# BarisYazici/deep-rl-grasping

Measured on NVIDIA H100. Metric: SAC grad-steps/sec (batch 256, 64x64 depth), higher is better.
Workload: dtype bf16x3 (fp32-faithful split, f32 accumulate)

## Files before the change

### deep-rl-grasping_b200/csrc/cg.cu

```cuda
#include <cuda_bf16.h>

#include <cstdio>
#include <cstdlib>

#include "cg.cuh"
#include "common.cuh"
#include "wgmma.cuh"

namespace b2g {
namespace {

constexpr int NEPI_WARPS = CG_EPI_WARPS, NPROD_WARPS = 2, PROD_WARP0 = NEPI_WARPS;
constexpr int NTHREADS = 32 * (NEPI_WARPS + 4);
constexpr int PROD_REGS = 40, CONS_REGS = 232;
constexpr int STG_BYTES = 2 * 64 * 16 * 4;

__device__ __forceinline__ uint32_t smem_u32(const void* p) { return (uint32_t)__cvta_generic_to_shared(p); }
__device__ __forceinline__ void mbar_init(uint32_t bar, uint32_t count) {
  asm volatile("mbarrier.init.shared::cta.b64 [%0], %1;" ::"r"(bar), "r"(count));
}
__device__ __forceinline__ void mbar_arrive(uint32_t bar) { asm volatile("mbarrier.arrive.shared::cta.b64 _, [%0];" ::"r"(bar) : "memory"); }
__device__ __forceinline__ void mbar_expect_tx(uint32_t bar, uint32_t bytes) {
  asm volatile("mbarrier.arrive.expect_tx.shared::cta.b64 _, [%0], %1;" ::"r"(bar), "r"(bytes) : "memory");
}
__device__ __forceinline__ void mbar_wait(uint32_t bar, uint32_t parity) {
  asm volatile(
      "{\n\t"
      ".reg .pred p;\n\t"
      "CG_WAIT:\n\t"
// ... 117 lines not shown
__device__ __forceinline__ void stamp_if(long long* dst, bool pred) {
  asm volatile(
      "{\n\t"
      ".reg .pred p;\n\t"
      ".reg .u64 t;\n\t"
      "mov.u64 t, %%clock64;\n\t"
      "setp.ne.u32 p, %1, 0;\n\t"
      "@p st.global.u64 [%0], t;\n\t"
      "}" ::"l"(dst), "r"((uint32_t)pred)
      : "memory");
}

template <int NT, int NPROD, int TRANS, int KS, class Body>
__device__ __forceinline__ void consume_tile(const CgProblem& P, const Tile& ti, uint32_t ring, uint32_t stg, int slot_bytes, int nstages, uint32_t& s,
                                             uint32_t& ph, uint64_t* bar_full, uint64_t* bar_empty, bool nomma, long long* ctrace, uint32_t& gc,
                                             Body&& body) {
  constexpr int NGRP = NPROD >= 6 ? 3 : (NPROD >= 3 ? 2 : 1);
  constexpr int NACC = NT / 2 * NGRP;
  const int tid = threadIdx.x, lane = tid & 31, warp = tid >> 5;
  const int wg = warp >> 2, wl = warp & 3, half = wl >> 1;
  float acc[NACC];
#pragma unroll
  for (int j = 0; j < NACC; ++j) acc[j] = 0.f;
  const uint32_t a_ps = (uint32_t)P.a_pstride, b_ps = (uint32_t)P.b_pstride, a_off = P.a_off, b_off = P.b_off, a_ks = P.a_kstep, b_ks = P.b_kstep;
  const uint32_t a_lbo = P.a_lbo, b_lbo = P.b_lbo;
  const uint32_t m_off = TRANS ? (uint32_t)wg * a_lbo : (uint32_t)wg * 8192u;
  uint32_t prev = 0;
  if (nomma) {
    for (int c = ti.c_begin; c < ti.c_end; ++c, ++gc) {
      mbar_wait(smem_u32(&bar_full[s]), (ph >> s) & 1u);
      mbar_arrive_if(smem_u32(&bar_empty[s]), lane == 0);
// ... 15 lines not shown
      stamp_if(tr + 5, stamp);
      prev = s;
      ph ^= 1u << s;
      if (++s == (uint32_t)nstages) s = 0;
    }
    wg_wait<0>();
    mbar_arrive_if(smem_u32(&bar_empty[prev]), lane == 0);
  }
  if constexpr (NGRP > 2) {
#pragma unroll
    for (int j = 0; j < NT / 2; ++j) acc[j] = acc[j] + (acc[j + NT / 2] + acc[j + NT]);
  } else if constexpr (NGRP > 1) {
#pragma unroll
    for (int j = 0; j < NT / 2; ++j) acc[j] = acc[j] + acc[j + NT / 2];
  }
  const int rrow = 32 * (wl & 1) + lane;
  const uint32_t wstg = stg + (uint32_t)wg * 4096u;
#pragma unroll
  for (int R = 0; R < (NT + 63) / 64; ++R) {
    float x[32];
#pragma unroll
    for (int t = 0; t < 4; ++t) {
      const int c0 = 64 * R + 16 * t;
      if (c0 < NT) {
        asm volatile("bar.sync %0, 128;" ::"r"(1 + wg) : "memory");
#pragma unroll
        for (int jj = 0; jj < 2; ++jj)
#pragma unroll
          for (int h = 0; h < 2; ++h) {
            const int row = 16 * wl + (lane >> 2) + 8 * h, chunk = 2 * jj + ((lane & 3) >> 1);
// ... 5 lines not shown
        if (half == (t >> 1)) {
#pragma unroll
          for (int cc = 0; cc < 4; ++cc) {
            const uint32_t a = wstg + (uint32_t)rrow * 64u + (uint32_t)((cc ^ ((rrow >> 1) & 3)) << 4);
            float* xd = x + 16 * (t & 1) + 4 * cc;
            asm volatile("ld.shared.v4.f32 {%0,%1,%2,%3}, [%4];" : "=f"(xd[0]), "=f"(xd[1]), "=f"(xd[2]), "=f"(xd[3]) : "r"(a));
          }
        }
      }
    }
    const int g = 2 * R + half;
    if (32 * g < NT) body(g, x);
  }
}

__global__ void __launch_bounds__(NTHREADS, 1)
cg_kernel(const __grid_constant__ CgPack pk, int nprob, int total_tiles, const CUtensorMap* __restrict__ maps, int max_stages,
          int dbg, long long* __restrict__ trace) {
  const CgProblem* __restrict__ probs = pk.p;
  extern __shared__ uint8_t smem_raw[];
  __shared__ __align__(8) uint64_t bar_full[CG_MAX_STAGES], bar_empty[CG_MAX_STAGES];
  const int tid = threadIdx.x, lane = tid & 31;
  const int warp = __shfl_sync(0xffffffffu, tid >> 5, 0);
  const int trace_cta = dbg >> 8;
  const bool dbg_noload = dbg & 1, dbg_nomma = dbg & 2, dbg_nostore = dbg & 4, dbg_nost = dbg & 16;
  if (tid == 0) {
    for (int s = 0; s < max_stages; ++s) { mbar_init(smem_u32(&bar_full[s]), 1); mbar_init(smem_u32(&bar_empty[s]), NEPI_WARPS); }
    asm volatile("fence.mbarrier_init.release.cluster;" ::: "memory");
  }
  __syncthreads();
  const uint32_t stg = (smem_u32(smem_raw) + 1023u) & ~1023u;
  const uint32_t ring = stg + STG_BYTES;
  pdl_trigger();
  pdl_wait();

  if (warp >= PROD_WARP0) {
    asm volatile("setmaxnreg.dec.sync.aligned.u32 %0;" ::"n"(PROD_REGS));
    const int pw = warp - PROD_WARP0;
    if (pw >= NPROD_WARPS) return;
    {
      uint32_t gc = 0, s = 0, ph = 0;
      int slot_bytes = 0, nstages = 1;
      Walker w;
      int n2 = 1, nloads = 0, planes = 0, tx = 0;
      const int* tab = nullptr;
      for (int tile = blockIdx.x; tile < total_tiles; tile += gridDim.x) {
        if (w.advance(probs, nprob, tile)) {
          const CgProblem& P = probs[w.p];
          n2 = P.n2; nloads = P.nloads; planes = P.planes; tx = P.tx_bytes; tab = P.tm_tab;
          if (P.slot_bytes != slot_bytes || P.nstages != nstages) {
            for (int q = 0; q < nstages; ++q) mbar_wait(smem_u32(&bar_empty[q]), ((ph >> q) & 1u) ^ 1u);
            slot_bytes = P.slot_bytes; nstages = P.nstages; s = 0;
          }
        }
        const Tile ti = w.tile(tile);
        const CgProblem& P = probs[ti.p];
        if (P.dep_ctr) {
          const int* __restrict__ ctr = P.dep_ctr;
          const int x0 = P.dep_by_chunk ? ti.c_begin : ti.tm, x1 = P.dep_by_chunk ? ti.c_end : ti.tm + 1;
          const int lo = x0 * P.dep_rows / P.dep_rows_tile, hi = min(P.dep_tiles - 1, (x1 * P.dep_rows - 1) / P.dep_rows_tile);
          const int expect = P.dep_expect * NEPI_WARPS;
          for (int j = lo + lane; j <= hi; j += 32) {
            int seen;
            do {
              asm volatile("ld.acquire.gpu.global.s32 %0, [%1];" : "=r"(seen) : "l"(ctr + j) : "memory");
              if (seen < expect) __nanosleep(100);
            } while (seen < expect);
          }
          __syncwarp();
          asm volatile("fence.proxy.async.global;" ::: "memory");
        }
// ... 36 lines not shown
                    for (int d = 2; d < 5; ++d) if (d == L.rank - 1) crd[d] = pl;
                    if ((j & (NPROD_WARPS - 1)) == pw && leader)
                      tma_load(sbase + (uint32_t)(pl * L.plane_stride + L.smem_off), maps + L.map, full, L.rank, crd);
                  }
                }
              }
            }
          }
          if (tr) { trace[gc * 8 + 2] = clock64(); trace[gc * 8 + 6] = ti.p * 100000 + ti.tm * 10 + ti.tn; }
          if (++c2 == n2) { c2 = 0; ++c1; }
          ph ^= 1u << s;
          if (++s == (uint32_t)nstages) s = 0;
        }
      }
    }
  } else {
    asm volatile("setmaxnreg.inc.sync.aligned.u32 %0;" ::"n"(CONS_REGS));
    const int ew = warp, half = (ew & 3) >> 1, q = 2 * (ew >> 2) + (ew & 1);
    uint32_t it = 0, s = 0, ph = 0, gc = 0;
    int slot_bytes = 0, nstages = 1;
    Walker w;
    long long* const ctrace = trace && blockIdx.x == trace_cta && ew == 0 ? trace : nullptr;
    const int r = q * 32 + lane;
    int epi = 0, rows_tile = 0, lim_rows = 0, umma_n = 0, out_planes = 0, grp_stride = 32, n_valid = 0;
    long long roff = 0, rmoff = 0, o_tm = 0, m_tm = 0;
    int ri0 = 0, ri1 = 0, grp_tab = 0;
    int shape = 0;
    const float* __restrict__ bias = nullptr;
    const uint16_t* __restrict__ mask = nullptr;
    for (int tile = blockIdx.x; tile < total_tiles; tile += gridDim.x) {
      if (w.advance(probs, nprob, tile)) {
        const CgProblem& Q = probs[w.p];
        epi = Q.epi; rows_tile = Q.rows_tile; lim_rows = Q.lim_rows; umma_n = Q.umma_n; out_planes = Q.out_planes;
        grp_stride = Q.grp_stride; n_valid = Q.n_valid; o_tm = Q.o_tm; m_tm = Q.m_tm; bias = Q.bias; mask = Q.mask;
        const int d0 = Q.d0, d1 = Q.d1;
        const int i0 = r % d0, i12 = r / d0, i1 = i12 % d1, i2 = i12 / d1;
        roff = Q.o_base + (long long)i0 * Q.o0 + (long long)i1 * Q.o1 + (long long)i2 * Q.o2;
        rmoff = Q.m_base + (long long)i0 * Q.m0 + (long long)i1 * Q.m1 + (long long)i2 * Q.m2;
        ri0 = i0; ri1 = i1; grp_tab = Q.grp_tab;
        shape = cg_shape_key(Q.umma_n, Q.nprod, Q.mn_major != 0, Q.ksteps);
        if (Q.slot_bytes != slot_bytes || Q.nstages != nstages) { slot_bytes = Q.slot_bytes; nstages = Q.nstages; s = 0; }
      }
      const Tile ti = w.tile(tile);
      if (ti.c_end <= ti.c_begin) continue;
      const CgProblem& P = probs[ti.p];
      const bool valid0 = r < rows_tile && ti.tm * rows_tile + r < lim_rows;
      const long long off0 = roff + (long long)ti.tm * o_tm, moff0 = rmoff + (long long)ti.tm * m_tm;
      const int n0 = ti.tn * umma_n, ngroups = umma_n >> 5;
      const bool tre = trace && blockIdx.x == trace_cta && ew == 0 && lane == 0 && it < 16;
      if (tre) trace[512 + it * 4 + 0] = clock64();
      const bool split_fin = P.ws != nullptr;
      float* __restrict__ wsrow = split_fin ? P.ws + ((size_t)(ti.tm * w.tiles_n + ti.tn) * 128 + r) * umma_n : nullptr;
      auto body = [&](int g, float (&x)[32], int pass) {
        const int ng = n0 + 32 * g;
        bool valid = valid0;
        long long off = off0, moff = moff0;
        if (grp_tab) {
          const int gg = ng >> 5;
          valid = valid0 && ri0 < P.grp_lim0[gg] && ri1 < P.grp_lim1[gg];
          off = off0 + P.grp_off[gg]; moff = moff0 + P.grp_moff[gg] - ng;
        }
        if (pass == 0 && split_fin) {
#pragma unroll
          for (int j = 0; j < 8; ++j)
            asm volatile("red.global.add.v4.f32 [%0], {%1,%2,%3,%4};" ::"l"(wsrow + 32 * g + 4 * j), "f"(x[4 * j]), "f"(x[4 * j + 1]), "f"(x[4 * j + 2]),
                         "f"(x[4 * j + 3])
                         : "memory");
          return;
        }
        const bool live = !dbg_nostore && ng < n_valid;
        float4 bv[8];
        uint4 mk[4];
        if (epi == CG_EPI_ACT && live) {
#pragma unroll
          for (int j = 0; j < 8; ++j) bv[j] = __ldg(reinterpret_cast<const float4*>(bias + (long long)(ng >> 5) * P.bias_grp) + j);
        }
        if (epi == CG_EPI_DGRAD && live) {
#pragma unroll
          for (int j = 0; j < 4; ++j) mk[j] = valid ? __ldg(reinterpret_cast<const uint4*>(mask + moff + ng) + j) : make_uint4(0, 0, 0, 0);
        }
        if (!live) return;
        if (epi == CG_EPI_RAW) {
          if (valid) {
            float* dst = P.out_f + off + (long long)(ng >> 5) * P.f_grp;
            if (P.atomic) {
#pragma unroll
              for (int j = 0; j < 8; ++j)
                asm volatile("red.global.add.v4.f32 [%0], {%1,%2,%3,%4};" ::"l"(dst + 4 * j), "f"(x[4 * j]), "f"(x[4 * j + 1]), "f"(x[4 * j + 2]),
                             "f"(x[4 * j + 3])
                             : "memory");
            } else {
#pragma unroll
              for (int j = 0; j < 8; ++j) *reinterpret_cast<float4*>(dst + 4 * j) = make_float4(x[4 * j], x[4 * j + 1], x[4 * j + 2], x[4 * j + 3]);
            }
          }
          return;
        }
        if (epi == CG_EPI_WGRAD) {
          if (valid) {
            const float sc = P.scale;
            float* dst = P.out_f + off + (long long)(ng >> 5) * P.f_grp;
            if (P.atomic) {
#pragma unroll
              for (int j = 0; j < 8; ++j)
                asm volatile("red.global.add.v4.f32 [%0], {%1,%2,%3,%4};" ::"l"(dst + 4 * j), "f"(x[4 * j] * sc), "f"(x[4 * j + 1] * sc),
                             "f"(x[4 * j + 2] * sc), "f"(x[4 * j + 3] * sc)
                             : "memory");
            } else {
#pragma unroll
              for (int j = 0; j < 8; ++j)
                *reinterpret_cast<float4*>(dst + 4 * j) = make_float4(x[4 * j] * sc, x[4 * j + 1] * sc, x[4 * j + 2] * sc, x[4 * j + 3] * sc);
              if (P.dp_n > 1) {
                const int i4 = (int)((dst - P.dp_gbase) >> 2), per4 = P.dp_per4;
#pragma unroll
                for (int j = 0; j < 8; ++j) {
                  const int owner = (i4 + j) / per4;
                  if (owner != P.dp_rank)
                    reinterpret_cast<float4*>(P.dp_recv[owner])[(size_t)P.dp_rank * per4 + (i4 + j - owner * per4)] =
                        make_float4(x[4 * j] * sc, x[4 * j + 1] * sc, x[4 * j + 2] * sc, x[4 * j + 3] * sc);
                }
              }
            }
          }
          return;
        }
        if (epi == CG_EPI_ACT) {
#pragma unroll
          for (int j = 0; j < 8; ++j) {
            x[4 * j] = fmaxf(x[4 * j] + bv[j].x, 0.f); x[4 * j + 1] = fmaxf(x[4 * j + 1] + bv[j].y, 0.f);
            x[4 * j + 2] = fmaxf(x[4 * j + 2] + bv[j].z, 0.f); x[4 * j + 3] = fmaxf(x[4 * j + 3] + bv[j].w, 0.f);
          }
          if (P.f0 > 0 && valid && !dbg_nost) {
            float* dst = P.out_f + (long long)ti.tm * P.f_tm + (long long)r * P.f0 + (long long)(ng >> 5) * P.f_grp;
#pragma unroll
            for (int j = 0; j < 8; ++j) *reinterpret_cast<float4*>(dst + 4 * j) = make_float4(x[4 * j], x[4 * j + 1], x[4 * j + 2], x[4 * j + 3]);
          }
        } else {
#pragma unroll
          for (int j = 0; j < 4; ++j) {
            const uint32_t w[4] = {mk[j].x, mk[j].y, mk[j].z, mk[j].w};
#pragma unroll
            for (int uu = 0; uu < 4; ++uu) {
              if (!(w[uu] & 0x00007FFFu)) x[8 * j + 2 * uu] = 0.f;
              if (!(w[uu] & 0x7FFF0000u)) x[8 * j + 2 * uu + 1] = 0.f;
            }
          }
          if (P.colsum) {
            float cs[32];
#pragma unroll
            for (int j = 0; j < 32; ++j) cs[j] = x[j];
#pragma unroll
            for (int wd = 16; wd >= 1; wd >>= 1) {
              const bool up = (lane & wd) != 0;
#pragma unroll
              for (int j = 0; j < wd; ++j) {
                const float send = up ? cs[j] : cs[j + wd], keep = up ? cs[j + wd] : cs[j];
                cs[j] = keep + __shfl_xor_sync(0xffffffffu, send, wd);
              }
            }
            atomicAdd(P.colsum + ((ng + lane) & P.colsum_mask), cs[0]);
          }
        }
        const long long gcol = grp_tab ? 0 : (long long)(ng >> 5) * grp_stride;
#pragma unroll 1
        for (int pl = 0; pl < out_planes; ++pl) {
          uint32_t pk[16];
#pragma unroll
          for (int j = 0; j < 16; ++j) {
            pk[j] = pack_bf16x2(x[2 * j], x[2 * j + 1]);
            x[2 * j] -= __uint_as_float(pk[j] << 16);
            x[2 * j + 1] -= __uint_as_float(pk[j] & 0xFFFF0000u);
          }
          if (valid && !dbg_nost) {
            uint16_t* dst = P.out_p[pl] + off + gcol;
#pragma unroll
            for (int j = 0; j < 4; ++j) *reinterpret_cast<uint4*>(dst + 8 * j) = make_uint4(pk[4 * j], pk[4 * j + 1], pk[4 * j + 2], pk[4 * j + 3]);
          }
        }
      };
      auto body0 = [&](int g, float (&x)[32]) { body(g, x, 0); };
#define CG_CONSUME(NT, NPROD, TRANS, KS) \
  consume_tile<NT, NPROD, TRANS, KS>(P, ti, ring, stg, slot_bytes, nstages, s, ph, bar_full, bar_empty, dbg_nomma, ctrace, gc, body0)
      switch (shape) {
        case cg_shape_key(32, 6, false, 4): CG_CONSUME(32, 6, 0, 4); break;
        case cg_shape_key(64, 6, false, 4): CG_CONSUME(64, 6, 0, 4); break;
        case cg_shape_key(64, 3, false, 4): CG_CONSUME(64, 3, 0, 4); break;
        case cg_shape_key(128, 3, false, 4): CG_CONSUME(128, 3, 0, 4); break;
        case cg_shape_key(64, 3, true, 4): CG_CONSUME(64, 3, 1, 4); break;
        case cg_shape_key(64, 3, true, 9): CG_CONSUME(64, 3, 1, 9); break;
        case cg_shape_key(128, 3, true, 4): CG_CONSUME(128, 3, 1, 4); break;
        default: __trap();
      }
#undef CG_CONSUME
      if (tre) trace[512 + it * 4 + 1] = clock64();
      bool last_arriver = !split_fin;
      if (split_fin) {
        __syncwarp();
        int old = 0;
        if (lane == 0) { __threadfence(); old = atomicAdd(P.ws_cnt + (ti.tm * w.tiles_n + ti.tn) * NEPI_WARPS + ew, 1); }
        old = __shfl_sync(0xffffffffu, old, 0);
        last_arriver = old == w.splits - 1;
        if (last_arriver) {
          __threadfence();
          if (lane == 0) P.ws_cnt[(ti.tm * w.tiles_n + ti.tn) * NEPI_WARPS + ew] = 0;
          for (int g = half; g < ngroups; g += 2) {
            float x[32];
#pragma unroll
            for (int j = 0; j < 8; ++j) {
              const float4 sum = __ldcg(reinterpret_cast<const float4*>(wsrow + 32 * g) + j);
              x[4 * j] = sum.x; x[4 * j + 1] = sum.y; x[4 * j + 2] = sum.z; x[4 * j + 3] = sum.w;
              __stcg(reinterpret_cast<float4*>(wsrow + 32 * g) + j, make_float4(0.f, 0.f, 0.f, 0.f));
            }
            body(g, x, 1);
          }
        }
      }
      __syncwarp();
      if (lane == 0 && P.done_ctr && last_arriver) {
        __threadfence();
        atomicAdd(P.done_ctr + ti.tm, 1);
      }
      if (tre) { trace[512 + it * 4 + 2] = clock64(); trace[512 + it * 4 + 3] = ti.p * 100000 + ti.tm * 10 + ti.tn; }
      ++it;
    }
  }
}

typedef CUresult (*EncodeTiledFn)(CUtensorMap*, CUtensorMapDataType, cuuint32_t, void*, const cuuint64_t*, const cuuint64_t*, const cuuint32_t*,
                                  const cuuint32_t*, CUtensorMapInterleave, CUtensorMapSwizzle, CUtensorMapL2promotion, CUtensorMapFloatOOBfill);
EncodeTiledFn g_encode = nullptr;

}

bool cg_shape_supported(int umma_n, int nprod, bool mn_major, int ksteps) {
  switch (cg_shape_key(umma_n, nprod, mn_major, ksteps)) {
    case cg_shape_key(32, 6, false, 4): case cg_shape_key(64, 6, false, 4): case cg_shape_key(64, 3, false, 4): case cg_shape_key(128, 3, false, 4):
    case cg_shape_key(64, 3, true, 4): case cg_shape_key(64, 3, true, 9): case cg_shape_key(128, 3, true, 4): return true;
    default: return false;
// ... 29 lines not shown
    for (int l = 0; l < P.nloads; ++l) {
      CgLoad& L = P.ld[l];
      L.plane_stride = L.smem_off >= P.b_off ? P.b_pstride : P.a_pstride;
      if (L.plane_box && L.box_bytes != L.plane_stride) return -2;
    }
    const int need = P.b_off + P.planes * P.b_pstride;
    P.slot_bytes = (need + 1023) / 1024 * 1024;
    slot = slot > P.slot_bytes ? slot : P.slot_bytes;
  }
  g.total_tiles = start;
  const int avail = smem_budget - 1024 ;
  g.slot_bytes = slot; g.nstages = 0;
  int ring = 0;
  for (int i = 0; i < g.n; ++i) {
    CgProblem& P = g.host[i];
    P.nstages = P.slot_bytes > 0 ? avail / P.slot_bytes : 0;
    if (P.nstages > CG_MAX_STAGES) P.nstages = CG_MAX_STAGES;
    if (P.nstages < 2) return -1;
    P.slot_bytes = avail / P.nstages / 1024 * 1024;
    g.nstages = g.nstages > P.nstages ? g.nstages : P.nstages;
    ring = ring > P.nstages * P.slot_bytes ? ring : P.nstages * P.slot_bytes;
  }
  g.ring_bytes = ring;
  return 0;
}

long long* g_cg_trace = nullptr;

cudaError_t cg_launch(const CgGroup& g, const CUtensorMap* dev_maps, int num_sms, cudaStream_t s, bool pdl, int debug_flags) {
  if (g.total_tiles <= 0 || (debug_flags & 8)) return cudaSuccess;
  static bool attr_set = false;
  if (!attr_set) {
    cudaError_t e = cudaFuncSetAttribute(cg_kernel, cudaFuncAttributeMaxDynamicSharedMemorySize, 226 * 1024);
    if (e != cudaSuccess) return e;
    attr_set = true;
  }
// ... 12 lines not shown
```

### deep-rl-grasping_b200/csrc/cg.cuh

```cuda
#pragma once
#include <cuda.h>
#include <cuda_runtime.h>
#include <stdint.h>

namespace b2g {

constexpr int CG_MAX_LOADS = 4;
constexpr int CG_MAX_PROBLEMS = 16;
constexpr int CG_MAX_STAGES = 8;
constexpr int CG_MAX_PLANES = 3;
constexpr int CG_EPI_WARPS = 8;

enum CgEpiKind : int {
  CG_EPI_ACT = 0,
  CG_EPI_RAW = 1,
  CG_EPI_DGRAD = 2,
  CG_EPI_WGRAD = 3,
};

struct CgLoad {
  int map;
  int rank;
  int box_bytes;
  int smem_off;
  int plane_stride;
  int plane_box;
  int c0[5];
  int d_tm[5], d_tn[5], d_c1[5], d_c2[5];
};

struct CgProblem {
  int tile_start, tiles_m, tiles_n, splits;
  int chunks, n2;
// ... 67 lines not shown
```

### deep-rl-grasping_b200/csrc/engine_v2.cu

```cuda
#include <cuda_bf16.h>

#include <algorithm>
#include <cstdio>
#include <cstdlib>
#include <cstring>

#include "sac_internal.cuh"

namespace b2g {
namespace {

struct Gather2Args {
  GatherArgs g;
  uint16_t* a1[2][3];
  uint16_t* fp[3][3];
  int KF, Ci, OH, OW;
};

__device__ __forceinline__ void split3(float y, uint16_t& p0, uint16_t& p1, uint16_t& p2) {
  const __nv_bfloat16 h0 = __float2bfloat16_rn(y);
  const float r1 = y - __bfloat162float(h0);
  const __nv_bfloat16 h1 = __float2bfloat16_rn(r1);
  const float r2 = r1 - __bfloat162float(h1);
  p0 = __bfloat16_as_ushort(h0); p1 = __bfloat16_as_ushort(h1); p2 = __bfloat16_as_ushort(__float2bfloat16_rn(r2));
// ... 244 lines not shown
int fuse_groups(b2g_sac* h, const std::vector<const CgGroup*>& parts, const std::vector<Wire>& wires, const char* name, std::vector<CgGroup>& out, int& n_ctr) {
  CgGroup f;
  std::vector<int> first(parts.size());
  for (size_t gi = 0; gi < parts.size(); ++gi) {
    first[gi] = f.n;
    for (int i = 0; i < parts[gi]->n; ++i) {
      if (f.n >= CG_MAX_PROBLEMS) return b2g_fail(B2G_EINVAL, std::string("engine v2: too many problems in fused launch ") + name);
      f.host[f.n++] = parts[gi]->host[i];
    }
  }
  std::vector<int> ctr_of(f.n, -1);
  for (const Wire& w : wires) {
    const int pi = first[w.prod] + w.pi, qi = first[w.cons] + w.ci;
    CgProblem& Pp = f.host[pi];
    CgProblem& Pc = f.host[qi];
    if (Pc.dep_ctr && ctr_of[pi] < 0) {
      ctr_of[pi] = (int)(intptr_t)Pc.dep_ctr - 1;
      Pc.dep_expect += Pp.ws ? Pp.tiles_n : Pp.tiles_n * Pp.splits;
      continue;
    }
    if (Pp.splits > 1 && (Pp.splits - 1) * ((Pp.chunks + Pp.splits - 1) / Pp.splits) >= Pp.chunks)
      return b2g_fail(B2G_EINVAL, std::string("engine v2: a wired split-K producer has an empty split (fused launch ") + name + ")");
    if (ctr_of[pi] < 0) { ctr_of[pi] = n_ctr; n_ctr += Pp.tiles_m; }
    Pc.dep_rows = w.dep_rows; Pc.dep_rows_tile = w.dep_rows_tile; Pc.dep_tiles = Pp.tiles_m; Pc.dep_by_chunk = w.by_chunk;
    Pc.dep_expect = Pp.ws ? Pp.tiles_n : Pp.tiles_n * Pp.splits;
    Pc.dep_ctr = (const int*)(intptr_t)(ctr_of[pi] + 1);
  }
  for (int i = 0; i < f.n; ++i) f.host[i].done_ctr = (int*)(intptr_t)(ctr_of[i] + 1);
  return push_group(h, out, f, name);
}
// ... 496 lines not shown
    g_cg_trace = s_trace_buf;
    const char* tc = getenv("B2G_CG_TRACE_CTA");
    cudaError_t e = cg_launch(g, h->v2.d_maps, h->num_sms - h->v2.sm_reserve, s, false, h->v2.dbg | ((tc ? atoi(tc) : 0) << 8));
    g_cg_trace = nullptr;
    if (e != cudaSuccess) return b2g_fail(B2G_ECUDA, cudaGetErrorString(e));
    static int shots = 0;
    if (shots++ == 3) {
      long long t[640];
      cudaStreamSynchronize(s);
      cudaMemcpy(t, s_trace_buf, sizeof(t), cudaMemcpyDeviceToHost);
      const long long t0 = t[0];
      fprintf(stderr, "cg trace %s (cycles; per chunk: prod wait_start wait_done issued | mma wait_start full_seen committed)\n", g.name);
      for (int i = 0; i < 64 && t[i * 8 + 2]; ++i)
        fprintf(stderr, "  chunk %2d (p %lld tm %lld): %7lld %7lld %7lld | %7lld %7lld %7lld\n", i, t[i * 8 + 6] / 100000, t[i * 8 + 6] % 100000 / 10, t[i * 8] - t0,
                t[i * 8 + 1] - t0, t[i * 8 + 2] - t0, t[i * 8 + 3] - t0, t[i * 8 + 4] - t0, t[i * 8 + 5] - t0);
      for (int i = 0; i < 16 && t[512 + i * 4 + 2]; ++i)
        fprintf(stderr, "  tile %d (p %lld tm %lld) epilogue: wait_start %7lld acc_full %7lld done %7lld | first group: ld issued %7lld ld done %7lld math done %7lld\n", i,
                t[512 + i * 4 + 3] / 100000, t[512 + i * 4 + 3] % 100000 / 10, t[512 + i * 4] - t0, t[512 + i * 4 + 1] - t0, t[512 + i * 4 + 2] - t0,
                t[576 + i * 4] - t0, t[576 + i * 4 + 1] - t0, t[576 + i * 4 + 2] - t0);
    }
    return 0;
  }
  CK(cg_launch(g, h->v2.d_maps, h->num_sms - h->v2.sm_reserve, s, pdl_enabled(), h->v2.dbg));
  return 0;
}

}
```

Baseline: 2109.

## Hand off ACT/DGRAD accumulators to a dedicated epilogue warpgroup via shared memory

Splits the consumer into two MMA warpgroups and a separate four-warp epilogue warpgroup. For ACT and DGRAD epilogues, the MMA warps dump accumulators into a swizzled shared-memory buffer and signal an mbarrier, so the next tile's MMA can overlap the bias/ReLU/mask/bf16-split store work. RAW and WGRAD epilogues stay in place. The cost is a reserved accumulator buffer that shrinks the TMA ring (fewer stages), register rebalancing across roles, and a single buffer that can stall MMA until the epilogue drains it.

```diff
diff --git a/deep-rl-grasping_b200/csrc/cg.cu b/deep-rl-grasping_b200/csrc/cg.cu
--- a/deep-rl-grasping_b200/csrc/cg.cu
+++ b/deep-rl-grasping_b200/csrc/cg.cu
@@ -10,9 +10,12 @@
 namespace b2g {
 namespace {
 
-constexpr int NEPI_WARPS = CG_EPI_WARPS, NPROD_WARPS = 2, PROD_WARP0 = NEPI_WARPS;
-constexpr int NTHREADS = 32 * (NEPI_WARPS + 4);
-constexpr int PROD_REGS = 40, CONS_REGS = 232;
+constexpr int NMMA_WARPS = 8, NEPI_WARPS = CG_EPI_WARPS, NPROD_WARPS = 2;
+constexpr int EPI_WARP0 = NMMA_WARPS, PROD_WARP0 = NMMA_WARPS + NEPI_WARPS;
+static_assert(NEPI_WARPS == 4, "the epilogue is one warpgroup: one row of the 128-row tile per lane");
+constexpr int NTHREADS = 32 * (PROD_WARP0 + 4);
+constexpr int MMA_REGS = 176, EPI_REGS = 136, PROD_REGS = 24;
+static_assert(2 * MMA_REGS + EPI_REGS + PROD_REGS <= 512, "register file");
 constexpr int STG_BYTES = 2 * 64 * 16 * 4;
 
 __device__ __forceinline__ uint32_t smem_u32(const void* p) { return (uint32_t)__cvta_generic_to_shared(p); }
@@ -160,7 +163,7 @@
 template <int NT, int NPROD, int TRANS, int KS, class Body>
 __device__ __forceinline__ void consume_tile(const CgProblem& P, const Tile& ti, uint32_t ring, uint32_t stg, int slot_bytes, int nstages, uint32_t& s,
                                              uint32_t& ph, uint64_t* bar_full, uint64_t* bar_empty, bool nomma, long long* ctrace, uint32_t& gc,
-                                             Body&& body) {
+                                             bool handoff, uint32_t acc_buf, uint32_t& nb, uint64_t* acc_full, uint64_t* acc_empty, Body&& body) {
   constexpr int NGRP = NPROD >= 6 ? 3 : (NPROD >= 3 ? 2 : 1);
   constexpr int NACC = NT / 2 * NGRP;
   const int tid = threadIdx.x, lane = tid & 31, warp = tid >> 5;
@@ -206,6 +209,22 @@
 #pragma unroll
     for (int j = 0; j < NT / 2; ++j) acc[j] = acc[j] + acc[j + NT / 2];
   }
+  if (handoff) {
+    mbar_wait(smem_u32(acc_empty), (nb & 1u) ^ 1u);
+    const uint32_t R = 64u * wg + 16u * wl + (uint32_t)(lane >> 2), sw = (uint32_t)(lane >> 2);
+    const uint32_t rowa = acc_buf + R * (uint32_t)(NT * 4) + (uint32_t)((lane & 1) * 8);
+#pragma unroll
+    for (int j = 0; j < NT / 8; ++j)
+#pragma unroll
+      for (int h = 0; h < 2; ++h) {
+        const uint32_t a = rowa + (uint32_t)h * (8u * NT * 4) + ((((uint32_t)(2 * j) + (uint32_t)((lane & 3) >> 1)) ^ sw) << 4);
+        asm volatile("st.shared.v2.f32 [%0], {%1,%2};" ::"r"(a), "f"(acc[4 * j + 2 * h]), "f"(acc[4 * j + 2 * h + 1]) : "memory");
+      }
+    __syncwarp();
+    mbar_arrive_if(smem_u32(acc_full), lane == 0);
+    ++nb;
+    return;
+  }
   const int rrow = 32 * (wl & 1) + lane;
   const uint32_t wstg = stg + (uint32_t)wg * 4096u;
 #pragma unroll
@@ -241,18 +260,32 @@
   }
 }
 
+struct RowOff {
+  long long roff = 0, rmoff = 0;
+  int ri0 = 0, ri1 = 0;
+  __device__ __forceinline__ void set(const CgProblem& Q, int r) {
+    const int d0 = Q.d0, d1 = Q.d1;
+    const int i0 = r % d0, i12 = r / d0, i1 = i12 % d1, i2 = i12 / d1;
+    roff = Q.o_base + (long long)i0 * Q.o0 + (long long)i1 * Q.o1 + (long long)i2 * Q.o2;
+    rmoff = Q.m_base + (long long)i0 * Q.m0 + (long long)i1 * Q.m1 + (long long)i2 * Q.m2;
+    ri0 = i0; ri1 = i1;
+  }
+};
+
 __global__ void __launch_bounds__(NTHREADS, 1)
 cg_kernel(const __grid_constant__ CgPack pk, int nprob, int total_tiles, const CUtensorMap* __restrict__ maps, int max_stages,
           int dbg, long long* __restrict__ trace) {
   const CgProblem* __restrict__ probs = pk.p;
   extern __shared__ uint8_t smem_raw[];
-  __shared__ __align__(8) uint64_t bar_full[CG_MAX_STAGES], bar_empty[CG_MAX_STAGES];
+  __shared__ __align__(8) uint64_t bar_full[CG_MAX_STAGES], bar_empty[CG_MAX_STAGES], acc_full, acc_empty;
   const int tid = threadIdx.x, lane = tid & 31;
   const int warp = __shfl_sync(0xffffffffu, tid >> 5, 0);
   const int trace_cta = dbg >> 8;
   const bool dbg_noload = dbg & 1, dbg_nomma = dbg & 2, dbg_nostore = dbg & 4, dbg_nost = dbg & 16;
   if (tid == 0) {
-    for (int s = 0; s < max_stages; ++s) { mbar_init(smem_u32(&bar_full[s]), 1); mbar_init(smem_u32(&bar_empty[s]), NEPI_WARPS); }
+    for (int s = 0; s < max_stages; ++s) { mbar_init(smem_u32(&bar_full[s]), 1); mbar_init(smem_u32(&bar_empty[s]), NMMA_WARPS); }
+    mbar_init(smem_u32(&acc_full), NMMA_WARPS);
+    mbar_init(smem_u32(&acc_empty), NEPI_WARPS);
     asm volatile("fence.mbarrier_init.release.cluster;" ::: "memory");
   }
   __syncthreads();
@@ -266,22 +299,29 @@
     const int pw = warp - PROD_WARP0;
     if (pw >= NPROD_WARPS) return;
     {
-      uint32_t gc = 0, s = 0, ph = 0;
+      uint32_t gc = 0, s = 0, ph = 0, nbuf = 0;
       int slot_bytes = 0, nstages = 1;
+      bool handoff = false;
       Walker w;
       int n2 = 1, nloads = 0, planes = 0, tx = 0;
       const int* tab = nullptr;
       for (int tile = blockIdx.x; tile < total_tiles; tile += gridDim.x) {
         if (w.advance(probs, nprob, tile)) {
           const CgProblem& P = probs[w.p];
-          n2 = P.n2; nloads = P.nloads; planes = P.planes; tx = P.tx_bytes; tab = P.tm_tab;
+          n2 = P.n2; nloads = P.nloads; planes = P.planes; tx = P.tx_bytes; tab = P.tm_tab; handoff = cg_epi_handoff(P.epi);
           if (P.slot_bytes != slot_bytes || P.nstages != nstages) {
             for (int q = 0; q < nstages; ++q) mbar_wait(smem_u32(&bar_empty[q]), ((ph >> q) & 1u) ^ 1u);
+            if (nbuf) {
+              mbar_wait(smem_u32(&acc_full), (nbuf - 1) & 1u);
+              mbar_wait(smem_u32(&acc_empty), (nbuf - 1) & 1u);
+              asm volatile("fence.proxy.async.shared::cta;" ::: "memory");
+            }
             slot_bytes = P.slot_bytes; nstages = P.nstages; s = 0;
           }
         }
         const Tile ti = w.tile(tile);
         const CgProblem& P = probs[ti.p];
+        if (handoff && ti.c_end > ti.c_begin) ++nbuf;
         if (P.dep_ctr) {
           const int* __restrict__ ctr = P.dep_ctr;
           const int x0 = P.dep_by_chunk ? ti.c_begin : ti.tm, x1 = P.dep_by_chunk ? ti.c_end : ti.tm + 1;
@@ -348,173 +388,80 @@
         }
       }
     }
-  } else {
-    asm volatile("setmaxnreg.inc.sync.aligned.u32 %0;" ::"n"(CONS_REGS));
-    const int ew = warp, half = (ew & 3) >> 1, q = 2 * (ew >> 2) + (ew & 1);
-    uint32_t it = 0, s = 0, ph = 0, gc = 0;
+  } else if (warp < NMMA_WARPS) {
+    asm volatile("setmaxnreg.inc.sync.aligned.u32 %0;" ::"n"(MMA_REGS));
+    const int q = 2 * (warp >> 2) + (warp & 1);
+    uint32_t it = 0, s = 0, ph = 0, gc = 0, nb = 0;
     int slot_bytes = 0, nstages = 1;
     Walker w;
-    long long* const ctrace = trace && blockIdx.x == trace_cta && ew == 0 ? trace : nullptr;
+    long long* const ctrace = trace && blockIdx.x == trace_cta && warp == 0 ? trace : nullptr;
     const int r = q * 32 + lane;
-    int epi = 0, rows_tile = 0, lim_rows = 0, umma_n = 0, out_planes = 0, grp_stride = 32, n_valid = 0;
-    long long roff = 0, rmoff = 0, o_tm = 0, m_tm = 0;
-    int ri0 = 0, ri1 = 0, grp_tab = 0;
-    int shape = 0;
-    const float* __restrict__ bias = nullptr;
-    const uint16_t* __restrict__ mask = nullptr;
+    int epi = 0, rows_tile = 0, lim_rows = 0, umma_n = 0, n_valid = 0, shape = 0;
+    bool handoff = false;
+    uint32_t acc_buf = 0;
+    long long o_tm = 0;
+    RowOff ro;
     for (int tile = blockIdx.x; tile < total_tiles; tile += gridDim.x) {
       if (w.advance(probs, nprob, tile)) {
         const CgProblem& Q = probs[w.p];
-        epi = Q.epi; rows_tile = Q.rows_tile; lim_rows = Q.lim_rows; umma_n = Q.umma_n; out_planes = Q.out_planes;
-        grp_stride = Q.grp_stride; n_valid = Q.n_valid; o_tm = Q.o_tm; m_tm = Q.m_tm; bias = Q.bias; mask = Q.mask;
-        const int d0 = Q.d0, d1 = Q.d1;
-        const int i0 = r % d0, i12 = r / d0, i1 = i12 % d1, i2 = i12 / d1;
-        roff = Q.o_base + (long long)i0 * Q.o0 + (long long)i1 * Q.o1 + (long long)i2 * Q.o2;
-        rmoff = Q.m_base + (long long)i0 * Q.m0 + (long long)i1 * Q.m1 + (long long)i2 * Q.m2;
-        ri0 = i0; ri1 = i1; grp_tab = Q.grp_tab;
+        epi = Q.epi; rows_tile = Q.rows_tile; lim_rows = Q.lim_rows; umma_n = Q.umma_n; n_valid = Q.n_valid; o_tm = Q.o_tm;
+        ro.set(Q, r);
         shape = cg_shape_key(Q.umma_n, Q.nprod, Q.mn_major != 0, Q.ksteps);
         if (Q.slot_bytes != slot_bytes || Q.nstages != nstages) { slot_bytes = Q.slot_bytes; nstages = Q.nstages; s = 0; }
+        handoff = cg_epi_handoff(epi);
+        acc_buf = ring + (uint32_t)(nstages * slot_bytes);
       }
       const Tile ti = w.tile(tile);
       if (ti.c_end <= ti.c_begin) continue;
       const CgProblem& P = probs[ti.p];
       const bool valid0 = r < rows_tile && ti.tm * rows_tile + r < lim_rows;
-      const long long off0 = roff + (long long)ti.tm * o_tm, moff0 = rmoff + (long long)ti.tm * m_tm;
-      const int n0 = ti.tn * umma_n, ngroups = umma_n >> 5;
-      const bool tre = trace && blockIdx.x == trace_cta && ew == 0 && lane == 0 && it < 16;
+      const long long off0 = ro.roff + (long long)ti.tm * o_tm;
+      const int n0 = ti.tn * umma_n;
+      const bool tre = trace && blockIdx.x == trace_cta && warp == 0 && lane == 0 && it < 16;
       if (tre) trace[512 + it * 4 + 0] = clock64();
-      const bool split_fin = P.ws != nullptr;
-      float* __restrict__ wsrow = split_fin ? P.ws + ((size_t)(ti.tm * w.tiles_n + ti.tn) * 128 + r) * umma_n : nullptr;
-      auto body = [&](int g, float (&x)[32], int pass) {
+      auto body = [&](int g, float (&x)[32]) {
         const int ng = n0 + 32 * g;
-        bool valid = valid0;
-        long long off = off0, moff = moff0;
-        if (grp_tab) {
-          const int gg = ng >> 5;
-          valid = valid0 && ri0 < P.grp_lim0[gg] && ri1 < P.grp_lim1[gg];
-          off = off0 + P.grp_off[gg]; moff = moff0 + P.grp_moff[gg] - ng;
-        }
-        if (pass == 0 && split_fin) {
+        if (dbg_nostore || ng >= n_valid || !valid0) return;
+        float* dst = P.out_f + off0 + (long long)(ng >> 5) * P.f_grp;
+        if (epi == CG_EPI_RAW) {
+          if (P.atomic) {
+#pragma unroll
+            for (int j = 0; j < 8; ++j)
+              asm volatile("red.global.add.v4.f32 [%0], {%1,%2,%3,%4};" ::"l"(dst + 4 * j), "f"(x[4 * j]), "f"(x[4 * j + 1]), "f"(x[4 * j + 2]),
+                           "f"(x[4 * j + 3])
+                           : "memory");
+          } else {
+#pragma unroll
+            for (int j = 0; j < 8; ++j) *reinterpret_cast<float4*>(dst + 4 * j) = make_float4(x[4 * j], x[4 * j + 1], x[4 * j + 2], x[4 * j + 3]);
+          }
+          return;
+        }
+        const float sc = P.scale;
+        if (P.atomic) {
 #pragma unroll
           for (int j = 0; j < 8; ++j)
-            asm volatile("red.global.add.v4.f32 [%0], {%1,%2,%3,%4};" ::"l"(wsrow + 32 * g + 4 * j), "f"(x[4 * j]), "f"(x[4 * j + 1]), "f"(x[4 * j + 2]),
-                         "f"(x[4 * j + 3])
+            asm volatile("red.global.add.v4.f32 [%0], {%1,%2,%3,%4};" ::"l"(dst + 4 * j), "f"(x[4 * j] * sc), "f"(x[4 * j + 1] * sc),
+                         "f"(x[4 * j + 2] * sc), "f"(x[4 * j + 3] * sc)
                          : "memory");
-          return;
-        }
-        const bool live = !dbg_nostore && ng < n_valid;
-        float4 bv[8];
-        uint4 mk[4];
-        if (epi == CG_EPI_ACT && live) {
-#pragma unroll
-          for (int j = 0; j < 8; ++j) bv[j] = __ldg(reinterpret_cast<const float4*>(bias + (long long)(ng >> 5) * P.bias_grp) + j);
-        }
-        if (epi == CG_EPI_DGRAD && live) {
-#pragma unroll
-          for (int j = 0; j < 4; ++j) mk[j] = valid ? __ldg(reinterpret_cast<const uint4*>(mask + moff + ng) + j) : make_uint4(0, 0, 0, 0);
-        }
-        if (!live) return;
-        if (epi == CG_EPI_RAW) {
-          if (valid) {
-            float* dst = P.out_f + off + (long long)(ng >> 5) * P.f_grp;
-            if (P.atomic) {
-#pragma unroll
-              for (int j = 0; j < 8; ++j)
-                asm volatile("red.global.add.v4.f32 [%0], {%1,%2,%3,%4};" ::"l"(dst + 4 * j), "f"(x[4 * j]), "f"(x[4 * j + 1]), "f"(x[4 * j + 2]),
-                             "f"(x[4 * j + 3])
-                             : "memory");
-            } else {
-#pragma unroll
-              for (int j = 0; j < 8; ++j) *reinterpret_cast<float4*>(dst + 4 * j) = make_float4(x[4 * j], x[4 * j + 1], x[4 * j + 2], x[4 * j + 3]);
+        } else {
+#pragma unroll
+          for (int j = 0; j < 8; ++j)
+            *reinterpret_cast<float4*>(dst + 4 * j) = make_float4(x[4 * j] * sc, x[4 * j + 1] * sc, x[4 * j + 2] * sc, x[4 * j + 3] * sc);
+          if (P.dp_n > 1) {
+            const int i4 = (int)((dst - P.dp_gbase) >> 2), per4 = P.dp_per4;
+#pragma unroll
+            for (int j = 0; j < 8; ++j) {
+              const int owner = (i4 + j) / per4;
+              if (owner != P.dp_rank)
+                reinterpret_cast<float4*>(P.dp_recv[owner])[(size_t)P.dp_rank * per4 + (i4 + j - owner * per4)] =
+                    make_float4(x[4 * j] * sc, x[4 * j + 1] * sc, x[4 * j + 2] * sc, x[4 * j + 3] * sc);
             }
           }
-          return;
-        }
-        if (epi == CG_EPI_WGRAD) {
-          if (valid) {
-            const float sc = P.scale;
-            float* dst = P.out_f + off + (long long)(ng >> 5) * P.f_grp;
-            if (P.atomic) {
-#pragma unroll
-              for (int j = 0; j < 8; ++j)
-                asm volatile("red.global.add.v4.f32 [%0], {%1,%2,%3,%4};" ::"l"(dst + 4 * j), "f"(x[4 * j] * sc), "f"(x[4 * j + 1] * sc),
-                             "f"(x[4 * j + 2] * sc), "f"(x[4 * j + 3] * sc)
-                             : "memory");
-            } else {
-#pragma unroll
-              for (int j = 0; j < 8; ++j)
-                *reinterpret_cast<float4*>(dst + 4 * j) = make_float4(x[4 * j] * sc, x[4 * j + 1] * sc, x[4 * j + 2] * sc, x[4 * j + 3] * sc);
-              if (P.dp_n > 1) {
-                const int i4 = (int)((dst - P.dp_gbase) >> 2), per4 = P.dp_per4;
-#pragma unroll
-                for (int j = 0; j < 8; ++j) {
-                  const int owner = (i4 + j) / per4;
-                  if (owner != P.dp_rank)
-                    reinterpret_cast<float4*>(P.dp_recv[owner])[(size_t)P.dp_rank * per4 + (i4 + j - owner * per4)] =
-                        make_float4(x[4 * j] * sc, x[4 * j + 1] * sc, x[4 * j + 2] * sc, x[4 * j + 3] * sc);
-                }
-              }
-            }
-          }
-          return;
-        }
-        if (epi == CG_EPI_ACT) {
-#pragma unroll
-          for (int j = 0; j < 8; ++j) {
-            x[4 * j] = fmaxf(x[4 * j] + bv[j].x, 0.f); x[4 * j + 1] = fmaxf(x[4 * j + 1] + bv[j].y, 0.f);
-            x[4 * j + 2] = fmaxf(x[4 * j + 2] + bv[j].z, 0.f); x[4 * j + 3] = fmaxf(x[4 * j + 3] + bv[j].w, 0.f);
-          }
-          if (P.f0 > 0 && valid && !dbg_nost) {
-            float* dst = P.out_f + (long long)ti.tm * P.f_tm + (long long)r * P.f0 + (long long)(ng >> 5) * P.f_grp;
-#pragma unroll
-            for (int j = 0; j < 8; ++j) *reinterpret_cast<float4*>(dst + 4 * j) = make_float4(x[4 * j], x[4 * j + 1], x[4 * j + 2], x[4 * j + 3]);
-          }
-        } else {
-#pragma unroll
-          for (int j = 0; j < 4; ++j) {
-            const uint32_t w[4] = {mk[j].x, mk[j].y, mk[j].z, mk[j].w};
-#pragma unroll
-            for (int uu = 0; uu < 4; ++uu) {
-              if (!(w[uu] & 0x00007FFFu)) x[8 * j + 2 * uu] = 0.f;
-              if (!(w[uu] & 0x7FFF0000u)) x[8 * j + 2 * uu + 1] = 0.f;
-            }
-          }
-          if (P.colsum) {
-            float cs[32];
-#pragma unroll
-            for (int j = 0; j < 32; ++j) cs[j] = x[j];
-#pragma unroll
-            for (int wd = 16; wd >= 1; wd >>= 1) {
-              const bool up = (lane & wd) != 0;
-#pragma unroll
-              for (int j = 0; j < wd; ++j) {
-                const float send = up ? cs[j] : cs[j + wd], keep = up ? cs[j + wd] : cs[j];
-                cs[j] = keep + __shfl_xor_sync(0xffffffffu, send, wd);
-              }
-            }
-            atomicAdd(P.colsum + ((ng + lane) & P.colsum_mask), cs[0]);
-          }
-        }
-        const long long gcol = grp_tab ? 0 : (long long)(ng >> 5) * grp_stride;
-#pragma unroll 1
-        for (int pl = 0; pl < out_planes; ++pl) {
-          uint32_t pk[16];
-#pragma unroll
-          for (int j = 0; j < 16; ++j) {
-            pk[j] = pack_bf16x2(x[2 * j], x[2 * j + 1]);
-            x[2 * j] -= __uint_as_float(pk[j] << 16);
-            x[2 * j + 1] -= __uint_as_float(pk[j] & 0xFFFF0000u);
-          }
-          if (valid && !dbg_nost) {
-            uint16_t* dst = P.out_p[pl] + off + gcol;
-#pragma unroll
-            for (int j = 0; j < 4; ++j) *reinterpret_cast<uint4*>(dst + 8 * j) = make_uint4(pk[4 * j], pk[4 * j + 1], pk[4 * j + 2], pk[4 * j + 3]);
-          }
         }
       };
-      auto body0 = [&](int g, float (&x)[32]) { body(g, x, 0); };
-#define CG_CONSUME(NT, NPROD, TRANS, KS) \
-  consume_tile<NT, NPROD, TRANS, KS>(P, ti, ring, stg, slot_bytes, nstages, s, ph, bar_full, bar_empty, dbg_nomma, ctrace, gc, body0)
+#define CG_CONSUME(NT, NPROD, TRANS, KS)                                                                                                      \
+  consume_tile<NT, NPROD, TRANS, KS>(P, ti, ring, stg, slot_bytes, nstages, s, ph, bar_full, bar_empty, dbg_nomma, ctrace, gc, handoff, acc_buf, \
+                                     nb, &acc_full, &acc_empty, body)
       switch (shape) {
         case cg_shape_key(32, 6, false, 4): CG_CONSUME(32, 6, 0, 4); break;
         case cg_shape_key(64, 6, false, 4): CG_CONSUME(64, 6, 0, 4); break;
@@ -526,7 +473,166 @@
         default: __trap();
       }
 #undef CG_CONSUME
-      if (tre) trace[512 + it * 4 + 1] = clock64();
+      if (tre) {
+        trace[512 + it * 4 + 1] = clock64();
+        trace[512 + it * 4 + 2] = handoff;
+        trace[512 + it * 4 + 3] = ti.p * 100000 + ti.tm * 10 + ti.tn;
+      }
+      ++it;
+    }
+  } else {
+    asm volatile("setmaxnreg.inc.sync.aligned.u32 %0;" ::"n"(EPI_REGS));
+    const int ew = warp - EPI_WARP0;
+    const int r = ew * 32 + lane;
+    uint32_t ne = 0;
+    int slot_bytes = 0, nstages = 1;
+    Walker w;
+    int epi = 0, rows_tile = 0, lim_rows = 0, umma_n = 0, out_planes = 0, grp_stride = 32, n_valid = 0, grp_tab = 0;
+    bool handoff = false;
+    uint32_t acc_buf = 0;
+    long long o_tm = 0, m_tm = 0;
+    RowOff ro;
+    const float* __restrict__ bias = nullptr;
+    const uint16_t* __restrict__ mask = nullptr;
+    for (int tile = blockIdx.x; tile < total_tiles; tile += gridDim.x) {
+      if (w.advance(probs, nprob, tile)) {
+        const CgProblem& Q = probs[w.p];
+        epi = Q.epi; rows_tile = Q.rows_tile; lim_rows = Q.lim_rows; umma_n = Q.umma_n; out_planes = Q.out_planes;
+        grp_stride = Q.grp_stride; n_valid = Q.n_valid; o_tm = Q.o_tm; m_tm = Q.m_tm; bias = Q.bias; mask = Q.mask; grp_tab = Q.grp_tab;
+        ro.set(Q, r);
+        if (Q.slot_bytes != slot_bytes || Q.nstages != nstages) { slot_bytes = Q.slot_bytes; nstages = Q.nstages; }
+        handoff = cg_epi_handoff(epi);
+        acc_buf = ring + (uint32_t)(nstages * slot_bytes);
+      }
+      const Tile ti = w.tile(tile);
+      if (ti.c_end <= ti.c_begin || !handoff) continue;
+      const CgProblem& P = probs[ti.p];
+      const bool valid0 = r < rows_tile && ti.tm * rows_tile + r < lim_rows;
+      const long long off0 = ro.roff + (long long)ti.tm * o_tm, moff0 = ro.rmoff + (long long)ti.tm * m_tm;
+      const int n0 = ti.tn * umma_n, ngroups = umma_n >> 5;
+      auto group_at = [&](int g, bool& valid, long long& off, long long& moff) {
+        const int ng = n0 + 32 * g;
+        valid = valid0; off = off0; moff = moff0;
+        if (grp_tab) {
+          const int gg = ng >> 5;
+          valid = valid0 && ro.ri0 < P.grp_lim0[gg] && ro.ri1 < P.grp_lim1[gg];
+          off = off0 + P.grp_off[gg]; moff = moff0 + P.grp_moff[gg] - ng;
+        }
+      };
+      const bool tre = trace && blockIdx.x == trace_cta && ew == 0 && lane == 0 && ne < 16;
+      if (tre) trace[576 + ne * 4 + 0] = clock64();
+      uint32_t mbits[4] = {0u, 0u, 0u, 0u};
+      if (epi == CG_EPI_DGRAD && !dbg_nostore) {
+#pragma unroll
+        for (int g = 0; g < 4; ++g) {
+          bool valid;
+          long long off, moff;
+          group_at(g, valid, off, moff);
+          const int ng = n0 + 32 * g;
+          if (g < ngroups && valid && ng < n_valid) {
+            uint4 mk[4];
+#pragma unroll
+            for (int j = 0; j < 4; ++j) mk[j] = __ldg(reinterpret_cast<const uint4*>(mask + moff + ng) + j);
+#pragma unroll
+            for (int j = 0; j < 4; ++j) {
+              const uint32_t wd[4] = {mk[j].x, mk[j].y, mk[j].z, mk[j].w};
+#pragma unroll
+              for (int uu = 0; uu < 4; ++uu) {
+                if (wd[uu] & 0x00007FFFu) mbits[g] |= 1u << (8 * j + 2 * uu);
+                if (wd[uu] & 0x7FFF0000u) mbits[g] |= 1u << (8 * j + 2 * uu + 1);
+              }
+            }
+          }
+        }
+      }
+      mbar_wait(smem_u32(&acc_full), ne & 1u);
+      if (tre) trace[576 + ne * 4 + 1] = clock64();
+      const bool split_fin = P.ws != nullptr;
+      float* __restrict__ wsrow = split_fin ? P.ws + ((size_t)(ti.tm * w.tiles_n + ti.tn) * 128 + r) * umma_n : nullptr;
+      auto body = [&](int g, float (&x)[32], int pass) {
+        const int ng = n0 + 32 * g;
+        bool valid;
+        long long off, moff;
+        group_at(g, valid, off, moff);
+        if (pass == 0 && split_fin) {
+#pragma unroll
+          for (int j = 0; j < 8; ++j)
+            asm volatile("red.global.add.v4.f32 [%0], {%1,%2,%3,%4};" ::"l"(wsrow + 32 * g + 4 * j), "f"(x[4 * j]), "f"(x[4 * j + 1]), "f"(x[4 * j + 2]),
+                         "f"(x[4 * j + 3])
+                         : "memory");
+          return;
+        }
+        const bool live = !dbg_nostore && ng < n_valid;
+        float4 bv[8];
+        if (epi == CG_EPI_ACT && live) {
+#pragma unroll
+          for (int j = 0; j < 8; ++j) bv[j] = __ldg(reinterpret_cast<const float4*>(bias + (long long)(ng >> 5) * P.bias_grp) + j);
+        }
+        if (!live) return;
+        if (epi == CG_EPI_ACT) {
+#pragma unroll
+          for (int j = 0; j < 8; ++j) {
+            x[4 * j] = fmaxf(x[4 * j] + bv[j].x, 0.f); x[4 * j + 1] = fmaxf(x[4 * j + 1] + bv[j].y, 0.f);
+            x[4 * j + 2] = fmaxf(x[4 * j + 2] + bv[j].z, 0.f); x[4 * j + 3] = fmaxf(x[4 * j + 3] + bv[j].w, 0.f);
+          }
+          if (P.f0 > 0 && valid && !dbg_nost) {
+            float* dst = P.out_f + (long long)ti.tm * P.f_tm + (long long)r * P.f0 + (long long)(ng >> 5) * P.f_grp;
+#pragma unroll
+            for (int j = 0; j < 8; ++j) *reinterpret_cast<float4*>(dst + 4 * j) = make_float4(x[4 * j], x[4 * j + 1], x[4 * j + 2], x[4 * j + 3]);
+          }
+        } else {
+          const uint32_t mb = g == 0 ? mbits[0] : g == 1 ? mbits[1] : g == 2 ? mbits[2] : mbits[3];
+#pragma unroll
+          for (int j = 0; j < 32; ++j)
+            if (!((mb >> j) & 1u)) x[j] = 0.f;
+          if (P.colsum) {
+            float cs[32];
+#pragma unroll
+            for (int j = 0; j < 32; ++j) cs[j] = x[j];
+#pragma unroll
+            for (int wd = 16; wd >= 1; wd >>= 1) {
+              const bool up = (lane & wd) != 0;
+#pragma unroll
+              for (int j = 0; j < wd; ++j) {
+                const float send = up ? cs[j] : cs[j + wd], keep = up ? cs[j + wd] : cs[j];
+                cs[j] = keep + __shfl_xor_sync(0xffffffffu, send, wd);
+              }
+            }
+            atomicAdd(P.colsum + ((ng + lane) & P.colsum_mask), cs[0]);
+          }
+        }
+        const long long gcol = grp_tab ? 0 : (long long)(ng >> 5) * grp_stride;
+#pragma unroll 1
+        for (int pl = 0; pl < out_planes; ++pl) {
+          uint32_t pk[16];
+#pragma unroll
+          for (int j = 0; j < 16; ++j) {
+            pk[j] = pack_bf16x2(x[2 * j], x[2 * j + 1]);
+            x[2 * j] -= __uint_as_float(pk[j] << 16);
+            x[2 * j + 1] -= __uint_as_float(pk[j] & 0xFFFF0000u);
+          }
+          if (valid && !dbg_nost) {
+            uint16_t* dst = P.out_p[pl] + off + gcol;
+#pragma unroll
+            for (int j = 0; j < 4; ++j) *reinterpret_cast<uint4*>(dst + 8 * j) = make_uint4(pk[4 * j], pk[4 * j + 1], pk[4 * j + 2], pk[4 * j + 3]);
+          }
+        }
+      };
+      const uint32_t rowa = acc_buf + (uint32_t)(r * umma_n * 4), sw = (uint32_t)(r & 7);
+      for (int g = 0; g < ngroups; ++g) {
+        float x[32];
+#pragma unroll
+        for (int cc = 0; cc < 8; ++cc) {
+          const uint32_t a = rowa + ((((uint32_t)(8 * g + cc)) ^ sw) << 4);
+          asm volatile("ld.shared.v4.f32 {%0,%1,%2,%3}, [%4];" : "=f"(x[4 * cc]), "=f"(x[4 * cc + 1]), "=f"(x[4 * cc + 2]), "=f"(x[4 * cc + 3]) : "r"(a));
+        }
+        if (g == ngroups - 1) {
+          __syncwarp();
+          mbar_arrive_if(smem_u32(&acc_empty), lane == 0);
+        }
+        body(g, x, 0);
+      }
+      ++ne;
       bool last_arriver = !split_fin;
       if (split_fin) {
         __syncwarp();
@@ -537,7 +643,7 @@
         if (last_arriver) {
           __threadfence();
           if (lane == 0) P.ws_cnt[(ti.tm * w.tiles_n + ti.tn) * NEPI_WARPS + ew] = 0;
-          for (int g = half; g < ngroups; g += 2) {
+          for (int g = 0; g < ngroups; ++g) {
             float x[32];
 #pragma unroll
             for (int j = 0; j < 8; ++j) {
@@ -554,8 +660,7 @@
         __threadfence();
         atomicAdd(P.done_ctr + ti.tm, 1);
       }
-      if (tre) { trace[512 + it * 4 + 2] = clock64(); trace[512 + it * 4 + 3] = ti.p * 100000 + ti.tm * 10 + ti.tn; }
-      ++it;
+      if (tre) { trace[576 + (ne - 1) * 4 + 2] = clock64(); trace[576 + (ne - 1) * 4 + 3] = ti.p * 100000 + ti.tm * 10 + ti.tn; }
     }
   }
 }
@@ -615,12 +720,14 @@
   int ring = 0;
   for (int i = 0; i < g.n; ++i) {
     CgProblem& P = g.host[i];
-    P.nstages = P.slot_bytes > 0 ? avail / P.slot_bytes : 0;
+    const int acc = cg_epi_handoff(P.epi) ? cg_acc_bytes(P.umma_n) : 0;
+    const int avail_ring = avail - acc;
+    P.nstages = P.slot_bytes > 0 ? avail_ring / P.slot_bytes : 0;
     if (P.nstages > CG_MAX_STAGES) P.nstages = CG_MAX_STAGES;
     if (P.nstages < 2) return -1;
-    P.slot_bytes = avail / P.nstages / 1024 * 1024;
+    P.slot_bytes = avail_ring / P.nstages / 1024 * 1024;
     g.nstages = g.nstages > P.nstages ? g.nstages : P.nstages;
-    ring = ring > P.nstages * P.slot_bytes ? ring : P.nstages * P.slot_bytes;
+    ring = ring > P.nstages * P.slot_bytes + acc ? ring : P.nstages * P.slot_bytes + acc;
   }
   g.ring_bytes = ring;
   return 0;
diff --git a/deep-rl-grasping_b200/csrc/cg.cuh b/deep-rl-grasping_b200/csrc/cg.cuh
--- a/deep-rl-grasping_b200/csrc/cg.cuh
+++ b/deep-rl-grasping_b200/csrc/cg.cuh
@@ -9,7 +9,7 @@
 constexpr int CG_MAX_PROBLEMS = 16;
 constexpr int CG_MAX_STAGES = 8;
 constexpr int CG_MAX_PLANES = 3;
-constexpr int CG_EPI_WARPS = 8;
+constexpr int CG_EPI_WARPS = 4;
 
 enum CgEpiKind : int {
   CG_EPI_ACT = 0,
@@ -17,6 +17,8 @@
   CG_EPI_DGRAD = 2,
   CG_EPI_WGRAD = 3,
 };
+__host__ __device__ constexpr bool cg_epi_handoff(int epi) { return epi == CG_EPI_ACT || epi == CG_EPI_DGRAD; }
+__host__ __device__ constexpr int cg_acc_bytes(int umma_n) { return 128 * umma_n * 4; }
 
 struct CgLoad {
   int map;
diff --git a/deep-rl-grasping_b200/csrc/engine_v2.cu b/deep-rl-grasping_b200/csrc/engine_v2.cu
--- a/deep-rl-grasping_b200/csrc/engine_v2.cu
+++ b/deep-rl-grasping_b200/csrc/engine_v2.cu
@@ -282,6 +282,8 @@
     const int pi = first[w.prod] + w.pi, qi = first[w.cons] + w.ci;
     CgProblem& Pp = f.host[pi];
     CgProblem& Pc = f.host[qi];
+    if (!cg_epi_handoff(Pp.epi))
+      return b2g_fail(B2G_EINVAL, std::string("engine v2: a wired producer must have an ACT or DGRAD epilogue (fused launch ") + name + ")");
     if (Pc.dep_ctr && ctr_of[pi] < 0) {
       ctr_of[pi] = (int)(intptr_t)Pc.dep_ctr - 1;
       Pc.dep_expect += Pp.ws ? Pp.tiles_n : Pp.tiles_n * Pp.splits;
@@ -808,10 +810,12 @@
       for (int i = 0; i < 64 && t[i * 8 + 2]; ++i)
         fprintf(stderr, "  chunk %2d (p %lld tm %lld): %7lld %7lld %7lld | %7lld %7lld %7lld\n", i, t[i * 8 + 6] / 100000, t[i * 8 + 6] % 100000 / 10, t[i * 8] - t0,
                 t[i * 8 + 1] - t0, t[i * 8 + 2] - t0, t[i * 8 + 3] - t0, t[i * 8 + 4] - t0, t[i * 8 + 5] - t0);
-      for (int i = 0; i < 16 && t[512 + i * 4 + 2]; ++i)
-        fprintf(stderr, "  tile %d (p %lld tm %lld) epilogue: wait_start %7lld acc_full %7lld done %7lld | first group: ld issued %7lld ld done %7lld math done %7lld\n", i,
-                t[512 + i * 4 + 3] / 100000, t[512 + i * 4 + 3] % 100000 / 10, t[512 + i * 4] - t0, t[512 + i * 4 + 1] - t0, t[512 + i * 4 + 2] - t0,
-                t[576 + i * 4] - t0, t[576 + i * 4 + 1] - t0, t[576 + i * 4 + 2] - t0);
+      for (int i = 0; i < 16 && t[512 + i * 4 + 1]; ++i)
+        fprintf(stderr, "  tile %d (p %lld tm %lld) mma: start %7lld sums out %7lld (%s)\n", i, t[512 + i * 4 + 3] / 100000, t[512 + i * 4 + 3] % 100000 / 10,
+                t[512 + i * 4] - t0, t[512 + i * 4 + 1] - t0, t[512 + i * 4 + 2] ? "handed off" : "in place");
+      for (int i = 0; i < 16 && t[576 + i * 4 + 2]; ++i)
+        fprintf(stderr, "  handoff %d (p %lld tm %lld) epilogue warpgroup: buffer wait %7lld start %7lld end %7lld\n", i, t[576 + i * 4 + 3] / 100000,
+                t[576 + i * 4 + 3] % 100000 / 10, t[576 + i * 4] - t0, t[576 + i * 4 + 1] - t0, t[576 + i * 4 + 2] - t0);
     }
     return 0;
   }
```

Result: faster. 2256 (median of 6 runs) (+6.9%).
